# VladimirRadenkovic/Image-inpainting-and-Super-Resolution-using-Diffusion-Models-and-Conditional-Flow-Matching

Measured on AMD Instinct MI355X. Metric: sampled images/sec (50-step, 32x32), higher is better.
Workload: dtype bf16

## Files before the change

### image-inpainting-and-super-resolution-using-diffusion-models-and-conditional-flow-matching_amd/csrc/capi.hip

```cpp
#include <cstring>
#include <vector>

#include "capi_internal.h"

static thread_local std::string g_err;
void mi355_set_error(const std::string& msg) { g_err = msg; }

const mi355_debug_config& mi355_default_debug() {
  static const mi355_debug_config d = [] { mi355_debug_config c; mi355_debug_defaults(&c); return c; }();
  return d;
}

extern "C" {

int mi355_version(void) { return 108; }
void mi355_debug_defaults(mi355_debug_config* c) {
  if (!c) return;
  std::memset(c, 0, sizeof(*c));
  c->conv_ws = 3; c->conv_small = 15; c->conv_min_wgs = 512; c->conv_stagger = 0; c->conv_ablate = 0; c->conv_spin_limit = 1 << 22;
  c->conv_time_reps = 0; c->gn_apply_max_hw = 64; c->gn_fuse = 1; c->l2_warm = 1; c->attn_fused = 1; c->gn_epilogue = 7; c->conv_pp = 109; c->conv_edge = 15;
}
int mi355_unet_status(mi355_unet* net, int clear) {
  if (!net) { mi355_set_error("null handle"); return -1; }
  return unet_status(net, clear);
}
const char* mi355_last_error(void) { return g_err.c_str(); }

int mi355_unet_param_count(const mi355_unet_config* cfg) {
  if (!cfg) { mi355_set_error("null config"); return -1; }
  std::vector<ParamInfo> p;
  int rc = unet_enumerate_params(*cfg, p);
  return rc ? rc : (int)p.size();
}

int mi355_unet_param_info(const mi355_unet_config* cfg, int index, char* name, int name_cap, int64_t shape[4], int* ndim) {
  if (!cfg || !name || !shape || !ndim) { mi355_set_error("null argument"); return -1; }
  std::vector<ParamInfo> p;
  if (int rc = unet_enumerate_params(*cfg, p)) return rc;
  MI355_REQUIRE(index >= 0 && index < (int)p.size(), -1, "param index out of range");
  MI355_REQUIRE((int)p[index].name.size() + 1 <= name_cap, -1, "name buffer too small");
  std::strcpy(name, p[index].name.c_str());
  *ndim = (int)p[index].shape.size();
  for (int i = 0; i < 4; ++i) shape[i] = i < *ndim ? p[index].shape[i] : 1;
  return 0;
}

int64_t mi355_unet_weight_bytes(const mi355_unet_config* cfg) {
  if (!cfg) { mi355_set_error("null config"); return -1; }
  return unet_weight_bytes(*cfg);
}

int mi355_unet_create(const mi355_unet_config* cfg, const float* const* params_host, int n_params, void* dev_weights,
                      int64_t dev_weights_bytes, void* stream, mi355_unet** out) {
  if (!cfg) { mi355_set_error("null config"); return -1; }
  return unet_build(*cfg, params_host, n_params, dev_weights, dev_weights_bytes, S(stream), out);
}

void mi355_unet_destroy(mi355_unet* net) { delete net; }

int mi355_unet_forward(mi355_unet* net, const float* x, int x_channels, const float* cond, int cond_channels, const float* t,
                       float* out, int batch, void* workspace, int64_t workspace_bytes, void* stream) {
  return unet_forward(net, x, x_channels, cond, cond_channels, t, out, batch, workspace, workspace_bytes, S(stream));
}

int mi355_unet_forward_t(mi355_unet* net, const float* x, int x_channels, const float* cond, int cond_channels, float t, float* out,
                         int batch, void* workspace, int64_t workspace_bytes, void* stream) {
  MI355_REQUIRE(net && workspace && batch > 0, -1, "unet_forward_t: bad argument");
  const WsLayout l = unet_ws_layout(net, batch);
  MI355_REQUIRE((int64_t)l.total <= workspace_bytes, -2, "unet_forward_t: workspace too small");
  float* tdev = reinterpret_cast<float*>(reinterpret_cast<char*>(workspace) + l.emb2);
  if (int rc = fill_launch(tdev, t, 1, S(stream))) return rc;
  return unet_forward(net, x, x_channels, cond, cond_channels, tdev, out, batch, workspace, workspace_bytes, S(stream), uniform_t_run());
}
// ... 215 lines not shown
```

### image-inpainting-and-super-resolution-using-diffusion-models-and-conditional-flow-matching_amd/csrc/common.h

```cpp
#pragma once
#include <hip/hip_runtime.h>
#include <stdint.h>
#include <atomic>
#include <cstring>
#include <string>

typedef __bf16 bf16;
typedef _Float16 f16;
typedef float f32x4 __attribute__((ext_vector_type(4)));
typedef float f32x2 __attribute__((ext_vector_type(2)));
typedef __bf16 bf16x8 __attribute__((ext_vector_type(8)));
typedef __bf16 bf16x4 __attribute__((ext_vector_type(4)));
typedef _Float16 f16x8 __attribute__((ext_vector_type(8)));
typedef _Float16 f16x4 __attribute__((ext_vector_type(4)));
typedef _Float16 f16x2 __attribute__((ext_vector_type(2)));
typedef uint32_t u32x4 __attribute__((ext_vector_type(4)));
typedef uint32_t u32x2 __attribute__((ext_vector_type(2)));

template <typename T> struct Elem;
template <> struct Elem<float> {
  static constexpr int CHUNK = 16;
  static constexpr int VEC = 4;
  static constexpr int DTYPE = 0;
};
// ... 106 lines not shown
  const uint64_t bit = 1ull << (dev & 63);
  if (done.load(std::memory_order_acquire) & bit) return 0;
  hipError_t e = hipFuncSetAttribute(reinterpret_cast<const void*>(kern), hipFuncAttributeMaxDynamicSharedMemorySize, 160 * 1024);
  if (e != hipSuccess) {
    (void)hipGetLastError();
    mi355_set_error(std::string(what) + ": hipFuncSetAttribute(MaxDynamicSharedMemorySize, 160 KB) failed: " + hipGetErrorString(e));
    return -3;
  }
  done.fetch_or(bit, std::memory_order_release);
  return 0;
}

__device__ __forceinline__ void l2_warm_wave(const void* p, uint32_t bytes) {
  const uint32_t rank = blockIdx.x >> 3, per = (gridDim.x + 7) >> 3, step = per * 64u * 128u;
  const char* base = reinterpret_cast<const char*>(p);
  uint32_t off = (rank * 64u + (threadIdx.x & 63)) * 128u;
  uint32_t v[16];
#pragma unroll
  for (int i = 0; i < 16; ++i, off += step) v[i] = *reinterpret_cast<const uint32_t*>(base + (off < bytes ? off : 0u));
#pragma unroll
  for (int i = 0; i < 16; ++i) asm volatile("" ::"v"(v[i]));
}

template <int NI>
struct GnPartial {
  f32x2 s2[NI], q2[NI];
  __device__ __forceinline__ GnPartial() {
#pragma unroll
    for (int i = 0; i < NI; ++i) { s2[i] = f32x2{0.f, 0.f}; q2[i] = f32x2{0.f, 0.f}; }
  }
  __device__ __forceinline__ void add(int ni, float v0, float v1, float v2, float v3, bool masked, float valid) {
    f32x2 lo = f32x2{v0, v1}, hi = f32x2{v2, v3};
    if (masked) { lo *= f32x2{valid, valid}; hi *= f32x2{valid, valid}; }
    s2[ni] += lo + hi;
    q2[ni] = lo * lo + q2[ni];
    q2[ni] = hi * hi + q2[ni];
  }
  static __device__ __forceinline__ float row_sum(float v) {
    v += __builtin_bit_cast(float, __builtin_amdgcn_update_dpp(0, __builtin_bit_cast(int, v), 0x140, 0xf, 0xf, false));
    v += __builtin_bit_cast(float, __builtin_amdgcn_update_dpp(0, __builtin_bit_cast(int, v), 0x141, 0xf, 0xf, false));
    v += __builtin_bit_cast(float, __builtin_amdgcn_update_dpp(0, __builtin_bit_cast(int, v), 0x4E, 0xf, 0xf, false));
    v += __builtin_bit_cast(float, __builtin_amdgcn_update_dpp(0, __builtin_bit_cast(int, v), 0xB1, 0xf, 0xf, false));
    return v;
  }
  __device__ __forceinline__ void store(float* dst, int lq, int lr) {
    float ms = 0.f, mq = 0.f;
#pragma unroll
    for (int ni = 0; ni < NI; ++ni) {
      const float ts = row_sum(s2[ni][0] + s2[ni][1]), tq = row_sum(q2[ni][0] + q2[ni][1]);
      if (lr == ni) { ms = ts; mq = tq; }
    }
    if (lr < NI) *reinterpret_cast<f32x2*>(dst + (size_t)(lr * 4 + lq) * 2) = f32x2{ms, mq};
  }
};
```

### image-inpainting-and-super-resolution-using-diffusion-models-and-conditional-flow-matching_amd/csrc/conv_pp.hip

```cpp
#include "conv_kargs.h"

#ifndef PP_IMPL
#define PP_IMPL "conv_pp.inc.h"
#endif
namespace {
#include PP_IMPL
}

int pp_route(const ConvDesc& d, const ConvPre& p, ConvRoute* r) {
  const Geo& g = p.g;
  const ConvKArgs& a = p.a;
  const int mode = p.K->conv_pp, Ho = g.Ho, Wo = g.Wo, Cout = d.Cout;
  if (!(mode & 3) || d.ks != 3 || g.G != 1 || g.bn_pack != 128 || d.out_mode != OUT_NHWC || g.stride != 1) return 1;
  if (p.has_pro && !d.pro_silu) return 1;
  if (a.nchunks < 2 || (a.nchunks & 1)) return 1;
  const bool up_ok = d.mode == CONV_UP2 && d.w_up2 && !d.wsplit && a.res_mode == RES_NONE;
  if (up_ok && (mode & 64) && !p.has_pro && Cout % 256 == 0 && !(Ho & 1) && !(Wo & 1) && Ho >= 32 && Wo >= 32) {
    const int tiles = ((d.Ws + 15) / 16) * ((d.Hs + 15) / 16);
    if ((mode & 3) >= 2 || 4 * d.N * tiles * (Cout / 256) >= ws_num_cus()) {
      r->kernel = CONV_K_PP; r->form = 2; r->w_up2 = 1;
      r->geom.BM = 256; r->geom.BN = 256; r->geom.lds_bytes = pp::D<0>::lds_bytes(false);
      const int slots = 4 * 2 * tiles;
      if (p.gn_ok && slots <= d.gn_slots_cap) r->gn_slots = slots;
      return 0;
    }
  }
  int cfg = -1;
  if (Cout % 256 == 0 && Wo >= 16 && Ho >= 16) cfg = 0;
  else if (Cout % 128 == 0 && (mode & 8) && Wo >= 32 && Ho >= 16) cfg = 1;
  if (cfg < 0) return 1;
  if (p.has_pro && !(mode & (cfg == 0 ? 4 : 16))) return 1;
  const int vw = cfg == 0 ? 16 : 32, bn = cfg == 0 ? 256 : 128;
  const int tiles = ((Wo + vw - 1) / vw) * ((Ho + 15) / 16);
  if ((mode & 3) < 2 && d.N * tiles * (Cout / bn) < ws_num_cus()) return 1;
  r->kernel = CONV_K_PP; r->form = cfg;
  r->geom.BM = cfg == 0 ? 256 : 512; r->geom.BN = bn;
  r->geom.lds_bytes = cfg == 0 ? pp::D<0>::lds_bytes(p.has_pro) : pp::D<1>::lds_bytes(p.has_pro);
  const bool act = cfg == 0 && Ho == 16 && Wo == 16 && (Cout == 256 || Cout == 512) && a.res_mode == RES_NONE;
  if (act && d.act_out && (p.K->gn_epilogue & 2) && d.act_out == d.out && !d.act_raw) r->act_done = 1;
  const int slots = (cfg == 0 ? 2 : 4) * tiles;
  if (!r->act_done && p.gn_ok && slots <= d.gn_slots_cap) r->gn_slots = slots;
  return 0;
}

int pp_launch(const ConvDesc& d, const ConvPre& p, const ConvRoute& r, hipStream_t stream) {
  ConvKArgs a = p.a;
  if (r.w_up2) {
    MI355_REQUIRE(d.w_up2, -1, "conv: the route asks for the collapsed up-sampling weights (conv_pack_weights_up2) and the description has none");
    a.w = d.w_up2; a.wbytes = (uint32_t)conv_packed_weight_bytes_up2(d.dtype, d.Cout, d.C0 + d.C1);
  }
  return dispatch_dtype(d.dtype, [&](auto t) { return launch_pp<decltype(t)>(a, r.form, stream); });
}
```

### image-inpainting-and-super-resolution-using-diffusion-models-and-conditional-flow-matching_amd/csrc/conv_pp.inc.h

```cpp
#ifndef PP_ABLATE
#define PP_ABLATE 0
#endif
#ifndef PP_TRACE_TAP0
#define PP_TRACE_TAP0 8
#endif
#ifdef CONV_STAMPS
#define PP_TRACE(k) if (tr_on) { const uint32_t ta = (uint32_t)(LDS_END + ((wave8 * 4 + (tr_tap - PP_TRACE_TAP0)) * 5 + (k)) * 4); uint32_t tv = (uint32_t)st_prev; asm volatile("v_mov_b32 %0, %2\n\tv_mov_b32 %1, %3\n\tds_write_b32 %0, %1" : "=&v"(tr_a), "=&v"(tr_v) : "s"(ta), "s"(tv) : "memory"); }
#define PP_TRACE_BYTES 2048
#else
#define PP_TRACE(k)
#define PP_TRACE_BYTES 0
#endif
namespace pp {
constexpr int NRING = 6, AHEAD = 5;
constexpr int ABUF = 512;
template <int CFG> struct G;
template <> struct G<0> {
  static constexpr int VW = 16, TH = 16, BN = 256, WM = 2, WROWS = 8, NWP = 2, NPW = 3;
  static constexpr int row(int mi) { return mi; }
  static constexpr int col(int mi) { (void)mi; return 0; }
};
template <> struct G<1> {
  static constexpr int VW = 32, TH = 16, BN = 128, WM = 4, WROWS = 4, NWP = 1, NPW = 5;
  static constexpr int row(int mi) { return mi >> 1; }
// ... 43 lines not shown
static_assert(S<0, 0>::younger(0) == 9 && S<0, 0>::younger(2) == 10 && S<0, 0>::younger(5) == 10 && S<0, 0>::younger(6) == 9 && S<0, 0>::younger(8) == 8, "window sums of the round-4 kernel");
static_assert(S<0, 0, 4>::ops_of(0) == 4 && S<0, 0, 4>::ops_of(1) == 3 && S<0, 0, 4>::ops_of(2) == 2 && S<0, 0, 4>::ops_of(3) == 2, "issue counts of the phase form");
static_assert(S<0, 0, 4>::yw(0) == 11 && S<0, 0, 4>::yw(1) == 11 && S<0, 0, 4>::yw(2) == 11 && S<0, 0, 4>::yw(3) == 11, "weight windows of the phase form");
static_assert(S<0, 0, 4>::younger(0) == 11 && S<0, 0, 4>::younger(2) == 11 && S<0, 0, 4>::younger(3) == 6, "window sums of the phase form");
static_assert(S<0, 0>::fill_yw(0) == 9 && S<1, 0>::fill_yw(0) == 5 && S<0, 0, 4>::fill_yw(0) == 10 && S<0, 0, 4>::fill_left() == 6 && S<0, 0, 4>::fill_yw(1) == 11,
              "fill windows: nine taps equal the steady state; four taps: the first L(0) has one operation fewer behind tap 1, so the fill waits for tap 1 too");
static_assert(S<0, 0, 4>::iss(2) < 4 - 1, "the last patch piece is issued before the L segment whose wait publishes the plane");
}

template <int N> __device__ __forceinline__ void pp_wait_vm() {
  static_assert(N >= 0 && N < 64, "vmcnt is 6 bits");
  asm volatile("" ::: "memory");
  __builtin_amdgcn_s_waitcnt((N & 15) | (7 << 4) | (15 << 8) | ((N >> 4) << 14));
  asm volatile("" ::: "memory");
}
__device__ __forceinline__ void pp_barrier() {
  asm volatile("" ::: "memory");
  __builtin_amdgcn_sched_barrier(0);
  __builtin_amdgcn_s_barrier();
  __builtin_amdgcn_sched_barrier(0);
  asm volatile("" ::: "memory");
}

template <int NV, typename T>
__device__ __forceinline__ void pp_pro_words(const uint32_t (&raw)[NV], const float* a, const float* b, uint32_t (&out)[NV], T) {
  float x[2 * NV], v[2 * NV], e[2 * NV];
#pragma unroll
  for (int i = 0; i < NV; ++i) { unpack2(raw[i], x[2 * i], x[2 * i + 1], T()); }
#pragma unroll
  for (int j = 0; j < 2 * NV; ++j) v[j] = a[j] * x[j] + b[j];
#pragma unroll
  for (int j = 0; j < 2 * NV; ++j) e[j] = -1.4426950408889634f * v[j];
#pragma unroll
  for (int j = 0; j < 2 * NV; ++j) e[j] = __builtin_amdgcn_exp2f(e[j]);
#pragma unroll
  for (int j = 0; j < 2 * NV; ++j) e[j] = 1.0f + e[j];
#pragma unroll
  for (int j = 0; j < 2 * NV; ++j) e[j] = __builtin_amdgcn_rcpf(e[j]);
#pragma unroll
  for (int j = 0; j < 2 * NV; ++j) v[j] = v[j] * e[j];
#pragma unroll
  for (int i = 0; i < NV; ++i) out[i] = pack2(v[2 * i], v[2 * i + 1], T());
}
template <int NV>
__device__ __forceinline__ void pp_pro_words(const uint32_t (&raw)[NV], const float* a, const float* b, uint32_t (&out)[NV], float) {
#pragma unroll
  for (int j = 0; j < NV; ++j) { const float v = a[j] * __builtin_bit_cast(float, raw[j]) + b[j]; out[j] = __builtin_bit_cast(uint32_t, v / (1.0f + expf(-v))); }
}

template <typename T, int CFG, int PRO, int ACT = 0, int UP = 0>
__global__ void __launch_bounds__(512, 2) conv3x3_pp_kernel(ConvKArgs p, int n_mt, int n_nt) {
  constexpr int TAPS = UP ? 4 : 9, KW = UP ? 2 : 3;
  static_assert(UP == 0 || (CFG == 0 && PRO == 0 && ACT == 0), "the phase form is the wide prologue-free kernel");
  using Dg = pp::D<CFG>;
  using Sc = pp::S<CFG, PRO, TAPS>;
  using E = Elem<T>;
  constexpr int NRING = pp::NRING, AHEAD = pp::AHEAD;
  constexpr int VW = Dg::VW, TH = Dg::TH, PW = Dg::PW, NPX = Dg::NPX, PLANE = Dg::PLANE, AROWB = Dg::AROWB, BN = Dg::BN, WTAP = Dg::WTAP;
  constexpr int OFF_PLANE = Dg::OFF_PLANE, OFF_AB = Dg::OFF_AB, NPW = Dg::NPW, NWP = Dg::NWP, WMN = Dg::WM, WROWS = Dg::WROWS;
  constexpr int CHUNK = E::CHUNK, ESZ = sizeof(T);
  constexpr int LDS_END = (int)Dg::lds_bytes(PRO, ACT), OFF_X = (int)Dg::lds_bytes(PRO);
  static_assert(ACT == 0 || CFG == 0, "the fused output GroupNorm needs whole images per tile: wide form at 16 x 16");
  (void)LDS_END; (void)NPX; (void)OFF_AB; (void)OFF_X;
  extern __shared__ __attribute__((aligned(16))) char smem[];

  const int lane = threadIdx.x & 63;
  const int wave8 = __builtin_amdgcn_readfirstlane(threadIdx.x >> 6);
  const int grp = wave8 >> 2;
  const int wm = CFG == 0 ? grp : wave8 >> 1, wn = CFG == 0 ? wave8 & 3 : wave8 & 1;
  const int lr = lane & 15, lq = lane >> 4;
  const int tpi = p.tiles_x * p.tiles_y;
  const int T9 = p.nchunks * TAPS;
  const int npt = p.N * tpi;
  const int ntp = ((n_mt + 7) / 8) * 8 * n_nt;
  auto decode = [&](int t, int& mt, int& nt) {
    const int per = 8 * n_nt, blk = t / per, r = t - blk * per;
    nt = r >> 3; mt = blk * 8 + (r & 7);
  };
  auto next_valid = [&](int t) {
    for (t += gridDim.x; t < ntp; t += gridDim.x) { int mt, nt; decode(t, mt, nt); if (mt < n_mt) break; }
    return t;
  };
  auto origin = [&](int mt, int& n0, int& y0, int& x0, int& ph) {
    ph = UP ? mt / npt : 0;
    if constexpr (UP != 0) mt -= ph * npt;
    const int ng = mt / tpi, rem = mt - ng * tpi;
    const int tyi = rem / p.tiles_x, txi = rem - tyi * p.tiles_x;
    n0 = ng; y0 = tyi * TH; x0 = txi * VW;
  };
  int t_first = (int)blockIdx.x - (int)gridDim.x;
  t_first = next_valid(t_first);
  if (t_first >= ntp) return;

  const __amdgpu_buffer_rsrc_t rs0 = __builtin_amdgcn_make_buffer_rsrc(const_cast<void*>(p.src0), 0, p.bytes0, 0x00020000);
  const __amdgpu_buffer_rsrc_t rs1 = __builtin_amdgcn_make_buffer_rsrc(const_cast<void*>(p.src1 ? p.src1 : p.src0), 0, p.bytes1, 0x00020000);
  const __amdgpu_buffer_rsrc_t rsw = __builtin_amdgcn_make_buffer_rsrc(const_cast<void*>(p.w), 0, p.wbytes, 0x00020000);
  const __amdgpu_buffer_rsrc_t rso = __builtin_amdgcn_make_buffer_rsrc(p.out, 0, (p.ablate & 1) ? 0u : p.obytes, 0x00020000);
  const __amdgpu_buffer_rsrc_t rsr = __builtin_amdgcn_make_buffer_rsrc(const_cast<void*>(p.res ? p.res : p.out), 0, p.rbytes, 0x00020000);
  const uint32_t abytes = PRO ? (uint32_t)p.N * (uint32_t)p.Cin * 4u : 0u;
  const __amdgpu_buffer_rsrc_t rsa = __builtin_amdgcn_make_buffer_rsrc(const_cast<float*>(PRO ? p.pro_a : p.bias), 0, abytes, 0x00020000);
  const __amdgpu_buffer_rsrc_t rsb = __builtin_amdgcn_make_buffer_rsrc(const_cast<float*>(PRO ? p.pro_b : p.bias), 0, abytes, 0x00020000);

  auto ws_base = [&](int t) {
    int mt, nt; decode(t, mt, nt);
    const int t128 = CFG == 0 ? 2 * nt + grp : nt;
    return (uint32_t)((UP ? 4 * t128 + mt / npt : t128) * T9) * 8192u;
  };
  uint32_t ws_soff = ws_base(t_first);
  const uint32_t wvo0 = (uint32_t)((CFG == 0 ? ((2 * wave8) & 7) : wave8) * 1024 + lane * 16), wvo1 = wvo0 + 1024u;
  auto issue_w_at = [&](int roff) {
    char* dst = smem + roff + (NWP * wave8) * 1024;
    __builtin_amdgcn_raw_ptr_buffer_load_lds(rsw, (__attribute__((address_space(3))) void*)dst, 16, wvo0, ws_soff, 0, 0);
    if constexpr (NWP == 2) __builtin_amdgcn_raw_ptr_buffer_load_lds(rsw, (__attribute__((address_space(3))) void*)(dst + 1024), 16, wvo1, ws_soff, 0, 0);
    ws_soff += 8192u;
  };
  auto issue_w = [&](auto ringc) { issue_w_at(decltype(ringc)::value * WTAP); };
  int ring_rd = 0, ring_wr = AHEAD * WTAP;
  (void)ring_rd; (void)ring_wr;
  constexpr bool KEYED = !(CFG == 0 && PRO == 0);
  uint32_t pvo0[6], pvo1[6];
  int pkey[6];
  int ps_n0 = 0;
  auto ps_setup = [&](int t) {
    int ln;
    asm volatile("v_mbcnt_lo_u32_b32 %0, -1, 0\n\tv_mbcnt_hi_u32_b32 %0, -1, %0" : "=v"(ln));
    asm volatile("" : "+s"(t));
    int mt, nt, n0, y0, x0, ph;
    decode(t, mt, nt);
    origin(mt, n0, y0, x0, ph);
    const int cy0 = y0 - 1 + (ph >> 1), cx0 = x0 - 1 + (ph & 1);
    const int Hb = UP ? p.Hs : p.Hc, Wb = UP ? p.Ws : p.Wc;
#pragma unroll
    for (int i = 0; i < NPW; ++i) {
      const int idx = 16 * (8 * i + wave8) + (ln >> 2);
      const int py = (int)(((float)idx + 0.5f) * (1.0f / (float)PW)), px = idx - py * PW;
      const int fqx = (ln & 3) ^ ((px >> 1) & 3);
      const int cy = cy0 + py, cx = cx0 + px;
      int sp = -1;
      if (idx < NPX && cy >= 0 && cy < Hb && cx >= 0 && cx < Wb) {
        if (UP == 0 && p.mode == CONV_UP2) sp = (n0 * p.Hs + (cy >> 1)) * p.Ws + (cx >> 1);
        else sp = (n0 * p.Hs + cy) * p.Ws + cx;
      }
      if constexpr (KEYED) {
        pkey[i] = sp >= 0 ? sp * 4 + fqx : -1;
      } else {
        pvo0[i] = sp >= 0 ? (uint32_t)sp * (uint32_t)(p.C0 * ESZ) + fqx * 16 : p.bytes0;
        pvo1[i] = sp >= 0 ? (uint32_t)sp * (uint32_t)(p.C1 * ESZ) + fqx * 16 : p.bytes1;
      }
    }
    if constexpr (PRO != 0) ps_n0 = n0;
  };
  ps_setup(t_first);
  auto issue_patch = [&](auto ic, auto planec, int sc) {
    constexpr int i = decltype(ic)::value, plane = decltype(planec)::value;
    const int cb = src_chunk(p, sc) * CHUNK;
    const bool first = cb < p.C0;
    const uint32_t so = (uint32_t)((first ? cb : cb - p.C0) * ESZ);
    char* dst = smem + OFF_PLANE + plane * PLANE + (8 * i + wave8) * 1024;
    uint32_t vo;
    if constexpr (KEYED) {
      const int k = pkey[i];
      const uint32_t rowb = (uint32_t)((first ? p.C0 : p.C1) * ESZ);
      vo = k >= 0 ? (uint32_t)(k >> 2) * rowb + (uint32_t)(k & 3) * 16u : (first ? p.bytes0 : p.bytes1);
    } else {
      vo = first ? pvo0[i] : pvo1[i];
    }
    __builtin_amdgcn_raw_ptr_buffer_load_lds(first ? rs0 : rs1, (__attribute__((address_space(3))) void*)dst, 16, vo, so, 0, 0);
  };
  auto issue_patch_at = [&](auto sc_tap, auto planec, int sc) {
    constexpr int S = decltype(sc_tap)::value;
    if constexpr (NPW > 0 && Sc::iss(0) == S) issue_patch(IC<0>(), planec, sc);
    if constexpr (NPW > 1 && Sc::iss(1 < NPW ? 1 : 0) == S) issue_patch(IC<1>(), planec, sc);
    if constexpr (NPW > 2 && Sc::iss(2 < NPW ? 2 : 0) == S) issue_patch(IC<2>(), planec, sc);
    if constexpr (NPW > 3 && Sc::iss(3 < NPW ? 3 : 0) == S) issue_patch(IC<3>(), planec, sc);
    if constexpr (NPW > 4 && Sc::iss(4 < NPW ? 4 : 0) == S) issue_patch(IC<4>(), planec, sc);
    if constexpr (NPW > 5 && Sc::iss(5 < NPW ? 5 : 0) == S) issue_patch(IC<5>(), planec, sc);
  };
  const uint32_t abvo = PRO ? ((uint32_t)lane < (uint32_t)CHUNK ? (uint32_t)lane * 4u : abytes) : 0u;
  auto issue_ab = [&](int sc) {
    if constexpr (PRO != 0) {
      const uint32_t so = (uint32_t)(ps_n0 * p.Cin + src_chunk(p, sc) * CHUNK) * 4u;
      char* dst = smem + OFF_AB + wave8 * pp::ABUF;
      __builtin_amdgcn_raw_ptr_buffer_load_lds(rsa, (__attribute__((address_space(3))) void*)dst, 4, abvo, so, 0, 0);
      __builtin_amdgcn_raw_ptr_buffer_load_lds(rsb, (__attribute__((address_space(3))) void*)(dst + 256), 4, abvo, so, 0, 0);
    }
  };
  struct TrOps { uint32_t raw[4]; float a[8], b[8]; int off; };
  auto tr_load = [&](auto ic, auto planec, TrOps& o) {
    constexpr int i = decltype(ic)::value, plane = decltype(planec)::value;
    int ln;
    asm volatile("v_mbcnt_lo_u32_b32 %0, -1, 0\n\tv_mbcnt_hi_u32_b32 %0, -1, %0" : "=v"(ln));
    o.off = OFF_PLANE + plane * PLANE + (8 * i + wave8) * 1024 + ((ln >> 2) << 6) + ((pkey[i] & 3) << 4);
    const char* abp = smem + OFF_AB + wave8 * pp::ABUF + (ln & 3) * (E::VEC * 4);
    const u32x4 r = *reinterpret_cast<const u32x4*>(smem + o.off);
    o.raw[0] = r[0]; o.raw[1] = r[1]; o.raw[2] = r[2]; o.raw[3] = r[3];
#pragma unroll
    for (int k = 0; k < E::VEC; k += 4) {
      const f32x4 av = *reinterpret_cast<const f32x4*>(abp + k * 4), bv = *reinterpret_cast<const f32x4*>(abp + 256 + k * 4);
      o.a[k] = av[0]; o.a[k + 1] = av[1]; o.a[k + 2] = av[2]; o.a[k + 3] = av[3];
      o.b[k] = bv[0]; o.b[k + 1] = bv[1]; o.b[k + 2] = bv[2]; o.b[k + 3] = bv[3];
    }
  };
  auto tr_finish = [&](auto ic, const TrOps& o) {
    constexpr int i = decltype(ic)::value;
    uint32_t ov[4];
    pp_pro_words<4>(o.raw, o.a, o.b, ov, T());
    if (pkey[i] >= 0) *reinterpret_cast<u32x4*>(smem + o.off) = u32x4{ov[0], ov[1], ov[2], ov[3]};
  };
  auto transform_piece = [&](auto ic, auto planec) {
    if constexpr (PRO != 0) { TrOps o; tr_load(ic, planec, o); tr_finish(ic, o); }
  };
  int a_base[3];
#pragma unroll
  for (int kx = 0; kx < 3; ++kx) a_base[kx] = OFF_PLANE + (wm * WROWS * PW + lr + kx) * 64 + 16 * (lq ^ (((lr + kx) >> 1) & 3));
  int b_base0 = (wn * 64 + lr) * 64 + 16 * (lq ^ ((lr >> 1) & 3));
  int b_base1 = b_base0 + 3 * WTAP;

  constexpr bool PAIR = E::DTYPE == 1;
  constexpr int NI = 4, NP2 = PAIR ? NI / 2 : NI, PSTEP = PAIR ? 32 : 16;
  f32x4 acc[8][NI];
  f32x4 cin[NI];
  auto cinit_load = [&](int t) {
    int mt, nt, n0, y0, x0, ph;
    decode(t, mt, nt);
    origin(mt, n0, y0, x0, ph);
#pragma unroll
    for (int ni = 0; ni < NI; ++ni) {
      const int co = nt * BN + wn * 64 + ni * 16 + 4 * lq;
      f32x4 v = f32x4{0.f, 0.f, 0.f, 0.f};
      if (p.bias) v = *reinterpret_cast<const f32x4*>(p.bias + co);
      if (p.emb) { const f32x4 e = *reinterpret_cast<const f32x4*>(p.emb + (size_t)n0 * p.emb_stride + co); v = f32x4{v[0] + e[0], v[1] + e[1], v[2] + e[2], v[3] + e[3]}; }
      cin[ni] = v;
    }
  };
  auto acc_init = [&]() {
#pragma unroll
    for (int mi = 0; mi < 8; ++mi)
#pragma unroll
      for (int ni = 0; ni < NI; ++ni) acc[mi][ni] = cin[ni];
  };

  constexpr int abl = PP_ABLATE;
  STAMP_DECL
  CLK_DECL
  cinit_load(t_first);
  issue_ab(0);
  issue_patch(IC<0>(), IC<0>(), 0); issue_patch(IC<1>(), IC<0>(), 0); issue_patch(IC<2>(), IC<0>(), 0);
  if constexpr (NPW > 3) issue_patch(IC<3>(), IC<0>(), 0);
  if constexpr (NPW > 4) issue_patch(IC<4>(), IC<0>(), 0);
  if constexpr (NPW > 5) issue_patch(IC<5>(), IC<0>(), 0);
  issue_w(IC<0>()); issue_w(IC<1>()); issue_w(IC<2>()); issue_w(IC<3>()); issue_w(IC<4>());
  acc_init();
  pp_wait_vm<Sc::fill_left()>();
  if constexpr (PRO != 0) {
    transform_piece(IC<0>(), IC<0>()); transform_piece(IC<1>(), IC<0>()); transform_piece(IC<2>(), IC<0>());
    if constexpr (NPW > 3) transform_piece(IC<3>(), IC<0>());
    if constexpr (NPW > 4) transform_piece(IC<4>(), IC<0>());
    if constexpr (NPW > 5) transform_piece(IC<5>(), IC<0>());
    asm volatile("s_waitcnt lgkmcnt(0)" ::: "memory");
  }
  pp_barrier();

  constexpr int EPI_STORES = 8 * NP2;
  const int extra0 = PAIR ? EPI_STORES * (p.res_mode != RES_NONE ? 2 : 1) : 0;
  int extra = 0;

  for (int t = t_first; t < ntp;) {
// ... 56 lines not shown
      uint32_t tr_a, tr_v;
#endif
      STAMP(0) PP_TRACE(0)
      constexpr int YW = Sc::yw(S), YP = Sc::yp(S), YY = YW < YP ? YW : YP;
      if constexpr (P == 0 && S < 4 && PAIR) {
        const int ex = UP ? (c == 0 ? extra : 0) : extra;
        if (ex == 0) pp_wait_vm<YY>();
        else if (ex == EPI_STORES) pp_wait_vm<(YW + EPI_STORES < YP ? YW + EPI_STORES : YP)>();
        else pp_wait_vm<(YW + 2 * EPI_STORES < YP ? YW + 2 * EPI_STORES : YP)>();
      } else {
        pp_wait_vm<YY>();
      }
      STAMP(1) PP_TRACE(1)
      pp_barrier();
      STAMP(2) PP_TRACE(2)
      __builtin_amdgcn_s_setprio(1);
      if constexpr (!(abl & 4)) {
#pragma unroll
        for (int mi = 0; mi < 8; ++mi)
#pragma unroll
          for (int ni = 0; ni < NI; ++ni) mma16(acc[mi][ni], bf[ni], af[mi], T());
      } else {
#pragma unroll
        for (int mi = 0; mi < 8; ++mi) asm volatile("" :: "v"(af[mi]));
#pragma unroll
        for (int ni = 0; ni < NI; ++ni) asm volatile("" :: "v"(bf[ni]));
      }
      __builtin_amdgcn_s_setprio(0);
      STAMP(3) PP_TRACE(3)
      if (!(last_of_tile && grp == 1)) pp_barrier();
      STAMP(4) PP_TRACE(4)
    };
    for (int c = 0; c < p.nchunks; c += 2) {
      const bool lastp = c + 2 >= p.nchunks;
      if constexpr (UP != 0) {
        tap(IC<0>(), IC<0>(), c, lastp); tap(IC<0>(), IC<1>(), c, lastp); tap(IC<0>(), IC<2>(), c, lastp); tap(IC<0>(), IC<3>(), c, lastp);
        tap(IC<1>(), IC<0>(), c + 1, lastp); tap(IC<1>(), IC<1>(), c + 1, lastp); tap(IC<1>(), IC<2>(), c + 1, lastp); tap(IC<1>(), IC<3>(), c + 1, lastp);
      } else {
      tap(IC<0>(), IC<0>(), c, lastp); tap(IC<0>(), IC<1>(), c, lastp); tap(IC<0>(), IC<2>(), c, lastp);
      tap(IC<0>(), IC<3>(), c, lastp); tap(IC<0>(), IC<4>(), c, lastp); tap(IC<0>(), IC<5>(), c, lastp);
      tap(IC<0>(), IC<6>(), c, lastp); tap(IC<0>(), IC<7>(), c, lastp); tap(IC<0>(), IC<8>(), c, lastp);
      tap(IC<1>(), IC<0>(), c + 1, lastp); tap(IC<1>(), IC<1>(), c + 1, lastp); tap(IC<1>(), IC<2>(), c + 1, lastp);
      tap(IC<1>(), IC<3>(), c + 1, lastp); tap(IC<1>(), IC<4>(), c + 1, lastp); tap(IC<1>(), IC<5>(), c + 1, lastp);
      tap(IC<1>(), IC<6>(), c + 1, lastp); tap(IC<1>(), IC<7>(), c + 1, lastp); tap(IC<1>(), IC<8>(), c + 1, lastp);
      }
    }

    cinit_load(t_nextc);
    const int co_w = nt * BN + wn * 64 + 4 * lq;
    const int co_s = PAIR ? nt * BN + wn * 64 + (lq & 1) * 16 + (lq >> 1) * 8 : co_w;
    GnPartial<NI> gp;
    const bool do_gn = p.gn_stats != nullptr;
    const int Hm = UP ? p.Hs : p.Ho, Wm = UP ? p.Ws : p.Wo;
    const bool gn_mask = ((Wm & (VW - 1)) | (Hm & (TH - 1))) != 0;
    auto epi_half = [&](auto hc, auto resc, auto gnc) {
      constexpr int h = decltype(hc)::value, GNM = decltype(gnc)::value;
      constexpr bool HAS_RES = decltype(resc)::value != 0;
      uint32_t ovo[4], rvo[4];
      float vm[4];
#pragma unroll
      for (int j = 0; j < 4; ++j) {
        const int y = y0 + wm * WROWS + Dg::row(h * 4 + j), x = x0 + Dg::col(h * 4 + j) + lr;
        const bool ok = y < Hm && x < Wm;
        vm[j] = ok ? 1.f : 0.f;
        const uint32_t opix = UP ? (uint32_t)((n0 * p.Ho + 2 * y + (ph >> 1)) * p.Wo + 2 * x + (ph & 1)) : (uint32_t)((n0 * p.Ho + y) * p.Wo + x);
        ovo[j] = ok ? (opix * (uint32_t)p.Cout + (uint32_t)co_s) * ESZ : p.obytes;
        uint32_t rpix = opix;
        if (p.res_mode == RES_UP2) rpix = (uint32_t)((n0 * p.Hr + (y >> 1)) * p.Wr + (x >> 1));
        rvo[j] = (ok && HAS_RES) ? (rpix * (uint32_t)p.Cout + (uint32_t)co_s) * ESZ : p.rbytes;
      }
      u32x4 rr[4][NP2];
      if constexpr (HAS_RES) {
#pragma unroll
        for (int j = 0; j < 4; ++j)
#pragma unroll
          for (int k = 0; k < NP2; ++k)
            rr[j][k] = __builtin_bit_cast(u32x4, __builtin_amdgcn_raw_buffer_load_b128(rsr, rvo[j] + k * PSTEP * ESZ, 0, 0));
      }
#pragma unroll
      for (int j = 0; j < 4; ++j) {
        const int mi = h * 4 + j;
        if constexpr (!PAIR) {
#pragma unroll
          for (int ni = 0; ni < NI; ++ni) {
            f32x4 o = acc[mi][ni];
            if constexpr (HAS_RES) {
              const f32x4 tt = __builtin_bit_cast(f32x4, rr[j][ni]);
              o = f32x4{o[0] + tt[0], o[1] + tt[1], o[2] + tt[2], o[3] + tt[3]};
            }
            if constexpr (GNM != 0) gp.add(ni, o[0], o[1], o[2], o[3], GNM == 2, vm[j]);
            __builtin_amdgcn_raw_buffer_store_b128(__builtin_bit_cast(u32x4, o), rso, ovo[j] + ni * 16 * ESZ, 0, 0);
          }
        } else {
#pragma unroll
          for (int k = 0; k < NP2; ++k) {
            float ra[4] = {0.f, 0.f, 0.f, 0.f}, rb[4] = {0.f, 0.f, 0.f, 0.f};
            if constexpr (HAS_RES) {
              const auto s0 = __builtin_amdgcn_permlane16_swap(rr[j][k][0], rr[j][k][2], false, false);
              const auto s1 = __builtin_amdgcn_permlane16_swap(rr[j][k][1], rr[j][k][3], false, false);
              const uint32_t xa[2] = {s0[0], s1[0]}, xb[2] = {s0[1], s1[1]};
#pragma unroll
              for (int q = 0; q < 2; ++q) {
                unpack2(xa[q], ra[2 * q], ra[2 * q + 1], T());
                unpack2(xb[q], rb[2 * q], rb[2 * q + 1], T());
              }
            }
            float va[4], vb[4];
#pragma unroll
            for (int q = 0; q < 4; ++q) {
              va[q] = HAS_RES ? acc[mi][2 * k][q] + ra[q] : acc[mi][2 * k][q];
              vb[q] = HAS_RES ? acc[mi][2 * k + 1][q] + rb[q] : acc[mi][2 * k + 1][q];
            }
            if constexpr (GNM != 0) {
              gp.add(2 * k, va[0], va[1], va[2], va[3], GNM == 2, vm[j]);
              gp.add(2 * k + 1, vb[0], vb[1], vb[2], vb[3], GNM == 2, vm[j]);
            }
            const u32x2 pa2 = pack4(va, T()), pb2 = pack4(vb, T());
            const auto w0 = __builtin_amdgcn_permlane16_swap(pa2[0], pb2[0], false, false);
// ... 37 lines not shown
      f32x4 ga[NI], gb[NI];
#pragma unroll
      for (int ni = 0; ni < NI; ++ni) {
        const float mean = gs[ni] * inv_cnt;
        const float var = fmaxf(gq[ni] * inv_cnt - mean * mean, 0.f);
        const float rstd = 1.0f / sqrtf(var + p.act_eps);
        const f32x4 g4 = *reinterpret_cast<const f32x4*>(p.act_gamma + co_w + ni * 16);
        const f32x4 b4 = *reinterpret_cast<const f32x4*>(p.act_beta + co_w + ni * 16);
#pragma unroll
        for (int j = 0; j < 4; ++j) {
          float a = rstd * g4[j];
          float b = b4[j] - mean * a;
          if (p.act_film) {
            const float* fpt = p.act_film + (size_t)n0 * p.act_film_stride + co_w + ni * 16 + j;
            const float sc = 1.0f + fpt[0], sh = fpt[p.Cout];
            a *= sc;
            b = b * sc + sh;
          }
          ga[ni][j] = a; gb[ni][j] = b;
        }
      }
      auto actv = [&](float v) {
        return p.act_silu ? (FASTA ? v * __builtin_amdgcn_rcpf(1.0f + __builtin_amdgcn_exp2f(-1.4426950408889634f * v)) : v / (1.0f + expf(-v))) : v;
      };
#pragma unroll
      for (int mi = 0; mi < 8; ++mi) {
        const int y = y0 + wm * WROWS + Dg::row(mi), x = x0 + Dg::col(mi) + lr;
        const uint32_t opix = (uint32_t)((n0 * p.Ho + y) * p.Wo + x);
        const uint32_t ovo = (opix * (uint32_t)p.Cout + (uint32_t)co_s) * ESZ;
        if constexpr (!PAIR) {
#pragma unroll
          for (int ni = 0; ni < NI; ++ni) {
            f32x4 o;
#pragma unroll
            for (int j = 0; j < 4; ++j) o[j] = actv(ga[ni][j] * acc[mi][ni][j] + gb[ni][j]);
            __builtin_amdgcn_raw_buffer_store_b128(__builtin_bit_cast(u32x4, o), rso, ovo + ni * 16 * ESZ, 0, 0);
          }
        } else {
#pragma unroll
          for (int k = 0; k < NP2; ++k) {
            float va[4], vb[4];
#pragma unroll
            for (int q = 0; q < 4; ++q) {
              va[q] = actv(ga[2 * k][q] * acc[mi][2 * k][q] + gb[2 * k][q]);
              vb[q] = actv(ga[2 * k + 1][q] * acc[mi][2 * k + 1][q] + gb[2 * k + 1][q]);
            }
            const u32x2 pa2 = pack4(va, T()), pb2 = pack4(vb, T());
            const auto w0 = __builtin_amdgcn_permlane16_swap(pa2[0], pb2[0], false, false);
            const auto w1 = __builtin_amdgcn_permlane16_swap(pa2[1], pb2[1], false, false);
            __builtin_amdgcn_raw_buffer_store_b128(u32x4{w0[0], w1[0], w0[1], w1[1]}, rso, ovo + k * PSTEP * ESZ, 0, 0);
          }
        }
      }
    } else if (p.res_mode != RES_NONE) {
      if (!do_gn) epi(IC<1>(), IC<0>()); else if (!gn_mask) epi(IC<1>(), IC<1>()); else epi(IC<1>(), IC<2>());
    } else {
      if (!do_gn) epi(IC<0>(), IC<0>()); else if (!gn_mask) epi(IC<0>(), IC<1>()); else epi(IC<0>(), IC<2>());
    }
    if (do_gn && ACT == 0) {
      const int rem = UP ? mt - ph * npt - n0 * tpi + ph * tpi : mt - n0 * tpi;
      gp.store(p.gn_stats + (((size_t)n0 * p.gn_slots + rem * WMN + wm) * (size_t)(p.Cout >> 2) + ((nt * BN + wn * 64) >> 2)) * 2, lq, lr);
    }
    acc_init();
    if constexpr (!PAIR) pp_wait_vm<0>();
    else if (p.ablate & 64) pp_wait_vm<0>();
    extra = (!PAIR || (p.ablate & 64)) ? 0 : extra0;
    STAMP(5)
    pp_barrier();
    STAMP(6)
    t = t_next;
  }
  pp_wait_vm<0>();
  STAMP_FLUSH
  CLK_FLUSH
#ifdef CONV_STAMPS
  if (p.dbg && blockIdx.x == 0 && lane < 20) p.dbg[2048 * 8 + wave8 * 20 + lane] = *reinterpret_cast<volatile uint32_t*>(smem + LDS_END + (wave8 * 20 + lane) * 4);
#endif
}

template <typename T, int CFG, int PRO, int ACT = 0, int UP = 0>
int launch_pp_k(ConvKArgs a, hipStream_t s) {
  using Dg = pp::D<CFG>;
  a.lvw = CFG == 0 ? 4 : 5; a.lth = 4; a.PW = Dg::PW; a.PH = Dg::PH; a.NP = Dg::NPX;
  const int Ht = UP ? a.Hs : a.Ho, Wt = UP ? a.Ws : a.Wo;
  a.tiles_x = (Wt + Dg::VW - 1) / Dg::VW; a.tiles_y = (Ht + Dg::TH - 1) / Dg::TH;
  const int n_mt = (UP ? 4 : 1) * a.N * a.tiles_x * a.tiles_y, n_nt = a.Cout / Dg::BN;
  if (int rc = mi355_allow_big_lds(conv3x3_pp_kernel<T, CFG, PRO, ACT, UP>, "conv3x3 (ping-pong)")) return rc;
  const int ntp = ((n_mt + 7) / 8) * 8 * n_nt, ncu = ws_num_cus();
  const int grid = ntp < ncu ? ntp : ncu;
  hipLaunchKernelGGL((conv3x3_pp_kernel<T, CFG, PRO, ACT, UP>), dim3(grid), dim3(512), Dg::lds_bytes(PRO, ACT) + PP_TRACE_BYTES, s, a, n_mt, n_nt);
  return 0;
}

template <typename T>
int launch_pp(const ConvKArgs& a, int cfg, hipStream_t s) {
  if (cfg == 2) return launch_pp_k<T, 0, 0, 0, 1>(a, s);
  if (a.act_out) return a.pro_a ? launch_pp_k<T, 0, 2, 1>(a, s) : launch_pp_k<T, 0, 0, 1>(a, s);
  if (a.pro_a) return cfg == 0 ? launch_pp_k<T, 0, 2>(a, s) : launch_pp_k<T, 1, 2>(a, s);
  return cfg == 0 ? launch_pp_k<T, 0, 0>(a, s) : launch_pp_k<T, 1, 0>(a, s);
}
```

### image-inpainting-and-super-resolution-using-diffusion-models-and-conditional-flow-matching_amd/csrc/unet_engine.hip

```cpp
#include "unet_engine.h"

#include <algorithm>
#include <cstring>
#include <map>

namespace {

inline size_t align_up(size_t v, size_t a) { return (v + a - 1) / a * a; }

enum BlockKind { BLK_CONV_IN, BLK_RES, BLK_ATTN, BLK_RESAMPLE_CONV, BLK_RESAMPLE, BLK_OUT };
struct Block {
  std::string prefix;
  int kind, cin, cout;
  int dir = 0;
  bool upsample = false;
  bool push = false, pop = false;
};
std::vector<Block> unet_blocks(const mi355_unet_config& cfg) {
  const int mc = cfg.model_channels, nl = cfg.n_channel_mult;
  auto has_attn = [&](int ds) { for (int i = 0; i < cfg.n_attention_ds; ++i) if (cfg.attention_ds[i] == ds) return true; return false; };
  std::vector<Block> out;
  auto add = [&](const std::string& prefix, int kind, int cin, int cout, int dir = 0) -> Block& {
    Block b; b.prefix = prefix; b.kind = kind; b.cin = cin; b.cout = cout; b.dir = dir;
    out.push_back(b);
// ... 102 lines not shown
    const float* p = P(name, {J, K});
    size_t o = alloc((size_t)J * K * 4);
    if (!dry && p) {
      float* d = reinterpret_cast<float*>(blob.data() + o);
      for (int j = 0; j < J; ++j) for (int k = 0; k < K; ++k) d[(size_t)k * J + j] = p[(size_t)j * K + k];
    }
    return o;
  }

  int tensor(int C, int H, int W) {
    PlanTensor t{C, H, W, false, net->act_elems_per_image};
    net->act_elems_per_image += align_up((size_t)C * H * W, 128);
    net->tensors.push_back(t);
    return (int)net->tensors.size() - 1;
  }
  const PlanTensor& T(int id) const { return net->tensors[id]; }

  int add_gn(int s0, int s1, const std::string& wname, const std::string& bname, int film_off, int apply_silu, bool may_apply = true) {
    const int max_hw = net->knobs.gn_apply_max_hw;
    const int C = T(s0).C + (s1 >= 0 ? T(s1).C : 0);
    PlanOp op; op.kind = OP_GN; op.src0 = s0; op.src1 = s1;
    op.gamma_off = put_f32(wname, {C}); op.beta_off = put_f32(bname, {C}); op.film_emb_off = film_off;
    if (cfg.differentiable) {
      op.gn_site = last_site = (int)net->site_C.size();
      net->site_C.push_back(C);
      net->site_off.push_back(net->site_floats_per_image);
      net->site_floats_per_image += (size_t)2 * C + 64;
    } else if (may_apply && T(s0).H * T(s0).W <= max_hw) { op.dst = tensor(C, T(s0).H, T(s0).W); op.pro_silu = apply_silu; }
    else {
      const int fuse = net->knobs.gn_fuse;
      const int C1 = s1 >= 0 ? T(s1).C : 0;
      if (fuse && (C / 32) % 4 == 0 && T(s0).C % 4 == 0 && C1 % 4 == 0) {
        op.fin_ok = 1;
        for (int s : {s0, s1}) {
          if (s < 0 || net->tensors[s].stats_cap) continue;
          PlanTensor& t = net->tensors[s];
          t.stats_cap = 4 * ((t.H * t.W + 63) / 64) + 8;
          t.stats_off_per_image = net->stats_floats_per_image;
          net->stats_floats_per_image += (size_t)t.stats_cap * (t.C / 4) * 2;
        }
      }
    }
    net->ops.push_back(op);
    if (C > net->max_gn_c) net->max_gn_c = C;
    return op.dst;
  }
  int add_conv(const std::string& prefix, int s0, int s1, int Cin_logical, int Cout, int ks, int mode, bool conv1d, int use_pro,
               int pro_silu, int emb_off, int res, int res_mode, int out_mode) {
    PlanOp op; op.kind = OP_CONV; op.src0 = s0; op.src1 = s1; op.mode = mode; op.ks = ks; op.Cout = Cout;
    op.w_off = put_conv(prefix + ".weight", Cout, Cin_logical, ks, conv1d);
    op.bias_off = put_f32(prefix + ".bias", {Cout});
    op.use_pro = use_pro; op.pro_silu = pro_silu; op.emb_off = emb_off; op.res = res; op.res_mode = res_mode; op.out_mode = out_mode;
    const int cin_t = T(s0).C + (s1 >= 0 ? T(s1).C : 0);
    if (mode == CONV_UP2 && ks == 3 && !conv1d && !use_pro && res < 0 && out_mode == OUT_NHWC && !cfg.differentiable && !net->wsplit && (net->knobs.conv_pp & 64) &&
        Cout % 256 == 0 && cin_t == Cin_logical && T(s0).H >= 16 && T(s0).W >= 16) {
      const float* pw = P(prefix + ".weight", {Cout, Cin_logical, ks, ks});
      op.has_wu = 1; op.wu_off = alloc(conv_packed_weight_bytes_up2(dtype, Cout, Cin_logical));
      if (!dry && pw) conv_pack_weights_up2(dtype, pw, Cout, Cin_logical, blob.data() + op.wu_off);
    }
    int Ho = T(s0).H, Wo = T(s0).W;
    if (mode == CONV_UP2) { Ho *= 2; Wo *= 2; }
    else if (mode == CONV_POOL2) { Ho /= 2; Wo /= 2; }
    else if (mode == CONV_STRIDE2) { Ho = (Ho - 1) / 2 + 1; Wo = (Wo - 1) / 2 + 1; }
    op.dst = out_mode == OUT_NHWC ? tensor(Cout, Ho, Wo) : -1;
    if (cfg.differentiable) {
      if (use_pro) op.gn_site = last_site;
      op.cin_pad = (int)align_up(T(s0).C + (s1 >= 0 ? T(s1).C : 0), 32);
      const float* pw = P(prefix + ".weight", conv1d ? std::vector<int64_t>{Cout, Cin_logical, 1} : std::vector<int64_t>{Cout, Cin_logical, ks, ks});
      op.wT_off = alloc(conv_packed_weight_bytes_dgrad(dtype, Cout, Cin_logical, ks, op.cin_pad));
      if (!dry && pw) conv_pack_weights_dgrad(dtype, pw, Cout, Cin_logical, ks, op.cin_pad, blob.data() + op.wT_off);
      const size_t hw_dgrad = mode == CONV_UP2 ? (size_t)Ho * Wo : (size_t)T(s0).H * T(s0).W;
      net->bwd_du_elems = std::max(net->bwd_du_elems, hw_dgrad * op.cin_pad);
      if (mode == CONV_STRIDE2) net->bwd_z_elems = std::max(net->bwd_z_elems, (size_t)T(s0).H * T(s0).W * Cout);
      net->bwd_tmp_elems = std::max(net->bwd_tmp_elems, (size_t)T(s0).H * T(s0).W * op.cin_pad);
    }
    net->ops.push_back(op);
    const double in_elems = (double)(T(s0).C + (s1 >= 0 ? T(s1).C : 0)) * T(s0).H * T(s0).W;
    net->conv_flops += 2.0 * Ho * Wo * (double)Cout * Cin_logical * ks * ks;
    net->act_bytes += (in_elems + (double)Cout * Ho * Wo) * esz;
    return op.dst;
  }

  int res_block(const std::string& p, int s0, int s1, int cin, int cout, bool up, bool down) {
    const bool film = cfg.use_scale_shift_norm != 0;
    const int ew = film ? 2 * cout : cout;
    const int eoff = emb_total;
    emb_parts.push_back({p + ".emb_layers.1", eoff, ew});
    emb_total += ew;
    P(p + ".emb_layers.1.weight", {ew, 4 * cfg.model_channels});
    P(p + ".emb_layers.1.bias", {ew});
    const int y1 = add_gn(s0, s1, p + ".in_layers.0.weight", p + ".in_layers.0.bias", -1, 1, !down);
    int h1;
    int res = s0, res_mode = up ? RES_UP2 : RES_SAME;
    if (down) {
      if (s1 >= 0) { err = "ResBlock(down) over a channel concat is not supported"; return -1; }
      PlanOp op; op.kind = OP_POOLAFF; op.src0 = s0; op.pro_silu = 1;
      op.dst = tensor(T(s0).C, T(s0).H / 2, T(s0).W / 2);
      if (cfg.differentiable) { op.gn_site = last_site; net->bwd_tmp_elems = std::max(net->bwd_tmp_elems, (size_t)T(s0).H * T(s0).W * T(s0).C); }
      net->ops.push_back(op);
      h1 = add_conv(p + ".in_layers.2", op.dst, -1, cin, cout, 3, CONV_UNIT, false, 0, 0, film ? -1 : eoff, -1, RES_NONE, OUT_NHWC);
      res = resample(s0, CONV_POOL2);
    } else {
      h1 = y1 >= 0 ? add_conv(p + ".in_layers.2", y1, -1, cin, cout, 3, up ? CONV_UP2 : CONV_UNIT, false, 0, 0, film ? -1 : eoff, -1, RES_NONE, OUT_NHWC)
                   : add_conv(p + ".in_layers.2", s0, s1, cin, cout, 3, up ? CONV_UP2 : CONV_UNIT, false, 1, 1, film ? -1 : eoff, -1, RES_NONE, OUT_NHWC);
    }
    const int y2 = add_gn(h1, -1, p + ".out_layers.0.weight", p + ".out_layers.0.bias", film ? eoff : -1, 1);
    if (cin != cout) {
      if (up || down) { err = "ResBlock(up/down) with a channel change is not supported"; return -1; }
// ... 687 lines not shown
```

Baseline: 1450.

## Add four-image tiled phase-form kernel for 8x8 upsample convs

Adds a UP==2 variant of the ping-pong conv kernel that packs four 8x8 source images into one 16x16 tile for the sub-pixel (phase) form of the upsample-by-2 3x3 conv. It enables this path by default through conv_pp bit 128 and packs the up2 weights for 8x8 inputs. Small-resolution upsample convs previously fell back to a less efficient path, so this aims to raise MFMA tile utilization there. The new tile decoding, LDS addressing and GroupNorm partial-stat layout add complexity and risk of correctness or stats-layout mismatches.

```diff
diff --git a/image-inpainting-and-super-resolution-using-diffusion-models-and-conditional-flow-matching_amd/csrc/capi.hip b/image-inpainting-and-super-resolution-using-diffusion-models-and-conditional-flow-matching_amd/csrc/capi.hip
--- a/image-inpainting-and-super-resolution-using-diffusion-models-and-conditional-flow-matching_amd/csrc/capi.hip
+++ b/image-inpainting-and-super-resolution-using-diffusion-models-and-conditional-flow-matching_amd/csrc/capi.hip
@@ -18,7 +18,7 @@
   if (!c) return;
   std::memset(c, 0, sizeof(*c));
   c->conv_ws = 3; c->conv_small = 15; c->conv_min_wgs = 512; c->conv_stagger = 0; c->conv_ablate = 0; c->conv_spin_limit = 1 << 22;
-  c->conv_time_reps = 0; c->gn_apply_max_hw = 64; c->gn_fuse = 1; c->l2_warm = 1; c->attn_fused = 1; c->gn_epilogue = 7; c->conv_pp = 109; c->conv_edge = 15;
+  c->conv_time_reps = 0; c->gn_apply_max_hw = 64; c->gn_fuse = 1; c->l2_warm = 1; c->attn_fused = 1; c->gn_epilogue = 7; c->conv_pp = 237; c->conv_edge = 15;
 }
 int mi355_unet_status(mi355_unet* net, int clear) {
   if (!net) { mi355_set_error("null handle"); return -1; }
diff --git a/image-inpainting-and-super-resolution-using-diffusion-models-and-conditional-flow-matching_amd/csrc/common.h b/image-inpainting-and-super-resolution-using-diffusion-models-and-conditional-flow-matching_amd/csrc/common.h
--- a/image-inpainting-and-super-resolution-using-diffusion-models-and-conditional-flow-matching_amd/csrc/common.h
+++ b/image-inpainting-and-super-resolution-using-diffusion-models-and-conditional-flow-matching_amd/csrc/common.h
@@ -182,4 +182,19 @@
     }
     if (lr < NI) *reinterpret_cast<f32x2*>(dst + (size_t)(lr * 4 + lq) * 2) = f32x2{ms, mq};
   }
-};
+  static __device__ __forceinline__ float half_row_sum(float v) {
+    v += __builtin_bit_cast(float, __builtin_amdgcn_update_dpp(0, __builtin_bit_cast(int, v), 0x141, 0xf, 0xf, false));
+    v += __builtin_bit_cast(float, __builtin_amdgcn_update_dpp(0, __builtin_bit_cast(int, v), 0x4E, 0xf, 0xf, false));
+    v += __builtin_bit_cast(float, __builtin_amdgcn_update_dpp(0, __builtin_bit_cast(int, v), 0xB1, 0xf, 0xf, false));
+    return v;
+  }
+  __device__ __forceinline__ void store_halves(float* dst, int lq, int lr, bool valid) {
+    float ms = 0.f, mq = 0.f;
+#pragma unroll
+    for (int ni = 0; ni < NI; ++ni) {
+      const float ts = half_row_sum(s2[ni][0] + s2[ni][1]), tq = half_row_sum(q2[ni][0] + q2[ni][1]);
+      if ((lr & 7) == ni) { ms = ts; mq = tq; }
+    }
+    if (valid && (lr & 7) < NI) *reinterpret_cast<f32x2*>(dst + (size_t)((lr & 7) * 4 + lq) * 2) = f32x2{ms, mq};
+  }
+};
diff --git a/image-inpainting-and-super-resolution-using-diffusion-models-and-conditional-flow-matching_amd/csrc/conv_pp.hip b/image-inpainting-and-super-resolution-using-diffusion-models-and-conditional-flow-matching_amd/csrc/conv_pp.hip
--- a/image-inpainting-and-super-resolution-using-diffusion-models-and-conditional-flow-matching_amd/csrc/conv_pp.hip
+++ b/image-inpainting-and-super-resolution-using-diffusion-models-and-conditional-flow-matching_amd/csrc/conv_pp.hip
@@ -22,6 +22,16 @@
       r->geom.BM = 256; r->geom.BN = 256; r->geom.lds_bytes = pp::D<0>::lds_bytes(false);
       const int slots = 4 * 2 * tiles;
       if (p.gn_ok && slots <= d.gn_slots_cap) r->gn_slots = slots;
+      return 0;
+    }
+  }
+  const bool act_fused = d.act_out && (p.K->gn_epilogue & 2) && d.act_out == d.out && !d.act_raw && (Cout == 256 || Cout == 512);
+  if (up_ok && (mode & 128) && !p.has_pro && !d.emb && !act_fused && Cout % 256 == 0 && d.Hs == 8 && d.Ws == 8) {
+    const int quads = (d.N + 3) / 4;
+    if ((mode & 3) >= 2 || 4 * quads * (Cout / 256) >= ws_num_cus()) {
+      r->kernel = CONV_K_PP; r->form = 3; r->w_up2 = 1;
+      r->geom.BM = 256; r->geom.BN = 256; r->geom.lds_bytes = pp::D<0>::lds_bytes(false);
+      if (p.gn_ok && 4 <= d.gn_slots_cap) r->gn_slots = 4;
       return 0;
     }
   }
diff --git a/image-inpainting-and-super-resolution-using-diffusion-models-and-conditional-flow-matching_amd/csrc/conv_pp.inc.h b/image-inpainting-and-super-resolution-using-diffusion-models-and-conditional-flow-matching_amd/csrc/conv_pp.inc.h
--- a/image-inpainting-and-super-resolution-using-diffusion-models-and-conditional-flow-matching_amd/csrc/conv_pp.inc.h
+++ b/image-inpainting-and-super-resolution-using-diffusion-models-and-conditional-flow-matching_amd/csrc/conv_pp.inc.h
@@ -119,6 +119,7 @@
 __global__ void __launch_bounds__(512, 2) conv3x3_pp_kernel(ConvKArgs p, int n_mt, int n_nt) {
   constexpr int TAPS = UP ? 4 : 9, KW = UP ? 2 : 3;
   static_assert(UP == 0 || (CFG == 0 && PRO == 0 && ACT == 0), "the phase form is the wide prologue-free kernel");
+  static_assert(UP >= 0 && UP <= 2, "UP: 0 nine taps, 1 phase form, 2 phase form on four-image tiles");
   using Dg = pp::D<CFG>;
   using Sc = pp::S<CFG, PRO, TAPS>;
   using E = Elem<T>;
@@ -138,7 +139,7 @@
   const int lr = lane & 15, lq = lane >> 4;
   const int tpi = p.tiles_x * p.tiles_y;
   const int T9 = p.nchunks * TAPS;
-  const int npt = p.N * tpi;
+  const int npt = UP == 2 ? (p.N + 3) >> 2 : p.N * tpi;
   const int ntp = ((n_mt + 7) / 8) * 8 * n_nt;
   auto decode = [&](int t, int& mt, int& nt) {
     const int per = 8 * n_nt, blk = t / per, r = t - blk * per;
@@ -153,7 +154,7 @@
     if constexpr (UP != 0) mt -= ph * npt;
     const int ng = mt / tpi, rem = mt - ng * tpi;
     const int tyi = rem / p.tiles_x, txi = rem - tyi * p.tiles_x;
-    n0 = ng; y0 = tyi * TH; x0 = txi * VW;
+    n0 = UP == 2 ? 4 * ng : ng; y0 = tyi * TH; x0 = txi * VW;
   };
   int t_first = (int)blockIdx.x - (int)gridDim.x;
   t_first = next_valid(t_first);
@@ -202,11 +203,15 @@
       const int idx = 16 * (8 * i + wave8) + (ln >> 2);
       const int py = (int)(((float)idx + 0.5f) * (1.0f / (float)PW)), px = idx - py * PW;
       const int fqx = (ln & 3) ^ ((px >> 1) & 3);
-      const int cy = cy0 + py, cx = cx0 + px;
+      int cy = cy0 + py, cx = cx0 + px, ni = n0;
+      if constexpr (UP == 2) {
+        const int by = py >= 9 ? 1 : 0, bx = px >= 9 ? 1 : 0;
+        cy -= 9 * by; cx -= 9 * bx; ni += 2 * by + bx;
+      }
       int sp = -1;
-      if (idx < NPX && cy >= 0 && cy < Hb && cx >= 0 && cx < Wb) {
+      if (idx < NPX && cy >= 0 && cy < Hb && cx >= 0 && cx < Wb && (UP != 2 || ni < p.N)) {
         if (UP == 0 && p.mode == CONV_UP2) sp = (n0 * p.Hs + (cy >> 1)) * p.Ws + (cx >> 1);
-        else sp = (n0 * p.Hs + cy) * p.Ws + cx;
+        else sp = (ni * p.Hs + cy) * p.Ws + cx;
       }
       if constexpr (KEYED) {
         pkey[i] = sp >= 0 ? sp * 4 + fqx : -1;
@@ -280,6 +285,13 @@
   int a_base[3];
 #pragma unroll
   for (int kx = 0; kx < 3; ++kx) a_base[kx] = OFF_PLANE + (wm * WROWS * PW + lr + kx) * 64 + 16 * (lq ^ (((lr + kx) >> 1) & 3));
+  if constexpr (UP == 2) {
+#pragma unroll
+    for (int kx = 0; kx < 3; ++kx) {
+      const int pcol = lr + (lr >> 3) + kx;
+      a_base[kx] = OFF_PLANE + (wm * (WROWS + 1) * PW + pcol) * 64 + 16 * (lq ^ ((pcol >> 1) & 3));
+    }
+  }
   int b_base0 = (wn * 64 + lr) * 64 + 16 * (lq ^ ((lr >> 1) & 3));
   int b_base1 = b_base0 + 3 * WTAP;
 
@@ -442,7 +454,7 @@
     GnPartial<NI> gp;
     const bool do_gn = p.gn_stats != nullptr;
     const int Hm = UP ? p.Hs : p.Ho, Wm = UP ? p.Ws : p.Wo;
-    const bool gn_mask = ((Wm & (VW - 1)) | (Hm & (TH - 1))) != 0;
+    const bool gn_mask = UP != 2 && ((Wm & (VW - 1)) | (Hm & (TH - 1))) != 0;
     auto epi_half = [&](auto hc, auto resc, auto gnc) {
       constexpr int h = decltype(hc)::value, GNM = decltype(gnc)::value;
       constexpr bool HAS_RES = decltype(resc)::value != 0;
@@ -450,10 +462,11 @@
       float vm[4];
 #pragma unroll
       for (int j = 0; j < 4; ++j) {
-        const int y = y0 + wm * WROWS + Dg::row(h * 4 + j), x = x0 + Dg::col(h * 4 + j) + lr;
-        const bool ok = y < Hm && x < Wm;
+        int y = y0 + wm * WROWS + Dg::row(h * 4 + j), x = x0 + Dg::col(h * 4 + j) + lr, ni = n0;
+        bool ok = y < Hm && x < Wm;
+        if constexpr (UP == 2) { y = Dg::row(h * 4 + j); x = lr & 7; ni = n0 + 2 * wm + (lr >> 3); ok = ni < p.N; }
         vm[j] = ok ? 1.f : 0.f;
-        const uint32_t opix = UP ? (uint32_t)((n0 * p.Ho + 2 * y + (ph >> 1)) * p.Wo + 2 * x + (ph & 1)) : (uint32_t)((n0 * p.Ho + y) * p.Wo + x);
+        const uint32_t opix = UP ? (uint32_t)((ni * p.Ho + 2 * y + (ph >> 1)) * p.Wo + 2 * x + (ph & 1)) : (uint32_t)((n0 * p.Ho + y) * p.Wo + x);
         ovo[j] = ok ? (opix * (uint32_t)p.Cout + (uint32_t)co_s) * ESZ : p.obytes;
         uint32_t rpix = opix;
         if (p.res_mode == RES_UP2) rpix = (uint32_t)((n0 * p.Hr + (y >> 1)) * p.Wr + (x >> 1));
@@ -597,11 +610,15 @@
           }
         }
       }
-    } else if (p.res_mode != RES_NONE) {
+    } else if (UP != 2 && p.res_mode != RES_NONE) {
       if (!do_gn) epi(IC<1>(), IC<0>()); else if (!gn_mask) epi(IC<1>(), IC<1>()); else epi(IC<1>(), IC<2>());
     } else {
       if (!do_gn) epi(IC<0>(), IC<0>()); else if (!gn_mask) epi(IC<0>(), IC<1>()); else epi(IC<0>(), IC<2>());
     }
+    if constexpr (UP == 2) {
+      const int ni = n0 + 2 * wm + (lr >> 3);
+      if (do_gn) gp.store_halves(p.gn_stats + (((size_t)ni * p.gn_slots + ph) * (size_t)(p.Cout >> 2) + ((nt * BN + wn * 64) >> 2)) * 2, lq, lr, ni < p.N);
+    } else
     if (do_gn && ACT == 0) {
       const int rem = UP ? mt - ph * npt - n0 * tpi + ph * tpi : mt - n0 * tpi;
       gp.store(p.gn_stats + (((size_t)n0 * p.gn_slots + rem * WMN + wm) * (size_t)(p.Cout >> 2) + ((nt * BN + wn * 64) >> 2)) * 2, lq, lr);
@@ -629,7 +646,7 @@
   a.lvw = CFG == 0 ? 4 : 5; a.lth = 4; a.PW = Dg::PW; a.PH = Dg::PH; a.NP = Dg::NPX;
   const int Ht = UP ? a.Hs : a.Ho, Wt = UP ? a.Ws : a.Wo;
   a.tiles_x = (Wt + Dg::VW - 1) / Dg::VW; a.tiles_y = (Ht + Dg::TH - 1) / Dg::TH;
-  const int n_mt = (UP ? 4 : 1) * a.N * a.tiles_x * a.tiles_y, n_nt = a.Cout / Dg::BN;
+  const int n_mt = UP == 2 ? 4 * ((a.N + 3) / 4) : (UP ? 4 : 1) * a.N * a.tiles_x * a.tiles_y, n_nt = a.Cout / Dg::BN;
   if (int rc = mi355_allow_big_lds(conv3x3_pp_kernel<T, CFG, PRO, ACT, UP>, "conv3x3 (ping-pong)")) return rc;
   const int ntp = ((n_mt + 7) / 8) * 8 * n_nt, ncu = ws_num_cus();
   const int grid = ntp < ncu ? ntp : ncu;
@@ -640,6 +657,7 @@
 template <typename T>
 int launch_pp(const ConvKArgs& a, int cfg, hipStream_t s) {
   if (cfg == 2) return launch_pp_k<T, 0, 0, 0, 1>(a, s);
+  if (cfg == 3) return launch_pp_k<T, 0, 0, 0, 2>(a, s);
   if (a.act_out) return a.pro_a ? launch_pp_k<T, 0, 2, 1>(a, s) : launch_pp_k<T, 0, 0, 1>(a, s);
   if (a.pro_a) return cfg == 0 ? launch_pp_k<T, 0, 2>(a, s) : launch_pp_k<T, 1, 2>(a, s);
   return cfg == 0 ? launch_pp_k<T, 0, 0>(a, s) : launch_pp_k<T, 1, 0>(a, s);
diff --git a/image-inpainting-and-super-resolution-using-diffusion-models-and-conditional-flow-matching_amd/csrc/unet_engine.hip b/image-inpainting-and-super-resolution-using-diffusion-models-and-conditional-flow-matching_amd/csrc/unet_engine.hip
--- a/image-inpainting-and-super-resolution-using-diffusion-models-and-conditional-flow-matching_amd/csrc/unet_engine.hip
+++ b/image-inpainting-and-super-resolution-using-diffusion-models-and-conditional-flow-matching_amd/csrc/unet_engine.hip
@@ -178,8 +178,9 @@
     op.bias_off = put_f32(prefix + ".bias", {Cout});
     op.use_pro = use_pro; op.pro_silu = pro_silu; op.emb_off = emb_off; op.res = res; op.res_mode = res_mode; op.out_mode = out_mode;
     const int cin_t = T(s0).C + (s1 >= 0 ? T(s1).C : 0);
-    if (mode == CONV_UP2 && ks == 3 && !conv1d && !use_pro && res < 0 && out_mode == OUT_NHWC && !cfg.differentiable && !net->wsplit && (net->knobs.conv_pp & 64) &&
-        Cout % 256 == 0 && cin_t == Cin_logical && T(s0).H >= 16 && T(s0).W >= 16) {
+    const bool up_shape = ((net->knobs.conv_pp & 64) && T(s0).H >= 16 && T(s0).W >= 16) || ((net->knobs.conv_pp & 128) && T(s0).H == 8 && T(s0).W == 8 && emb_off < 0);
+    if (mode == CONV_UP2 && ks == 3 && !conv1d && !use_pro && res < 0 && out_mode == OUT_NHWC && !cfg.differentiable && !net->wsplit && up_shape &&
+        Cout % 256 == 0 && cin_t == Cin_logical) {
       const float* pw = P(prefix + ".weight", {Cout, Cin_logical, ks, ks});
       op.has_wu = 1; op.wu_off = alloc(conv_packed_weight_bytes_up2(dtype, Cout, Cin_logical));
       if (!dry && pw) conv_pack_weights_up2(dtype, pw, Cout, Cin_logical, blob.data() + op.wu_off);
```

Result: no change. 1459, median of 6 (+0.6%).
